# ZhengdiYu/Arbitrary-Hands-3D-Reconstruction

Measured on AMD Instinct MI355X. Metric: frames/sec (2-hand mesh) at 512x512 batch-64; vertex L2 vs ref, higher is better.
Workload: dtype f32; 1 GPU; configs[2]: synthetic 512x512 RGB batch=64 per GPU, HRNet-W32 backbone, fp32; frames_per_gpu=64, global_batch=64, parallelism=frame-sharded x1, gather=none (one rank), contexts_in_turn=2

## Files before the change

### arbitrary-hands-3d-reconstruction_amd/csrc/pair1x1.hip

```cpp
#include "conv_frame.h"

namespace acrmi {

constexpr int PR_C1 = 64, PR_C2 = 256, PR_C3 = 64;
constexpr int PR_PIX = 256;
constexpr int PR_MT = 1, PR_WAVES = PR_PIX / (32 * PR_MT);
constexpr int PR_LDS_FLOATS = PR_C2 * PR_C1 + PR_C3 * PR_C2 + PR_C2 + PR_C3;

__global__ __launch_bounds__(PR_WAVES * 64, 1) void pair1x1_kernel(const float* __restrict__ t2, int t2_cs, int t2_coff,
                                                         const float* __restrict__ x, int x_cs, int x_coff,
                                                         float* __restrict__ y, int y_cs, int y_coff,
                                                         float* __restrict__ t, int t_cs, int t_coff,
                                                         const float* __restrict__ wpk, long npix) {
  extern __shared__ f32x4 smem4[];
  const f32x4* a1 = smem4;
  const f32x4* a2 = smem4 + PR_C2 * PR_C1 / 4;
  const f32x4* b3 = a2 + PR_C3 * PR_C2 / 4;
  const f32x4* b1 = b3 + PR_C2 / 4;
  const int tid = threadIdx.x, lane = tid & 63, wave = tid >> 6;
  const int li = lane & 31, lh = lane >> 5;
  for (int i = tid; i < PR_LDS_FLOATS / 4; i += PR_WAVES * 64) smem4[i] = reinterpret_cast<const f32x4*>(wpk)[i];

  const long items = (npix + PR_PIX - 1) / PR_PIX;
  auto pix_of = [&](long item, int p) -> long { return item * PR_PIX + 32 * PR_MT * wave + 32 * p + li; };
  f32x4 bq[PR_MT][8], bn[PR_MT][8];
  auto request_t2 = [&](long item, f32x4 (&dst)[PR_MT][8]) {
#pragma unroll
    for (int p = 0; p < PR_MT; ++p) {
      long px = pix_of(item, p);
      px = px < npix ? px : npix - 1;
      const f32x4* src = reinterpret_cast<const f32x4*>(t2 + (size_t)px * t2_cs + t2_coff + 32 * lh);
#pragma unroll
      for (int q = 0; q < 8; ++q) dst[p][q] = src[q];
    }
  };
  long item = blockIdx.x;
  if (item < items) request_t2(item, bq);
  __syncthreads();
  for (; item < items; item += gridDim.x) {
    const long nitem = item + gridDim.x;
    if (nitem < items) request_t2(nitem, bn);
    long px[PR_MT];
    bool ok[PR_MT];
#pragma unroll
    for (int p = 0; p < PR_MT; ++p) {
      px[p] = pix_of(item, p);
      ok[p] = px[p] < npix;
      px[p] = ok[p] ? px[p] : npix - 1;
    }
    f32x16 acc2[PR_MT][2];
    const f32x16 zero = {0.f, 0.f, 0.f, 0.f, 0.f, 0.f, 0.f, 0.f, 0.f, 0.f, 0.f, 0.f, 0.f, 0.f, 0.f, 0.f};
#pragma unroll 1
    for (int c = 0; c < 8; ++c) {
      f32x4 rv[PR_MT][4];
#pragma unroll
      for (int p = 0; p < PR_MT; ++p) {
        const float* xr = x + (size_t)px[p] * x_cs + x_coff + 32 * c + 4 * lh;
#pragma unroll
        for (int g = 0; g < 4; ++g) rv[p][g] = *reinterpret_cast<const f32x4*>(xr + 8 * g);
      }
      f32x16 acc1[PR_MT];
#pragma unroll
      for (int s4 = 0; s4 < 8; ++s4) {
        const f32x4 af = a1[(c * 8 + s4) * 64 + lane];
#pragma unroll
        for (int e = 0; e < 4; ++e)
#pragma unroll
          for (int p = 0; p < PR_MT; ++p) {
            if (s4 == 0 && e == 0) acc1[p] = __builtin_amdgcn_mfma_f32_32x32x2f32(af[e], bq[p][s4][e], zero, 0, 0, 0);
            else acc1[p] = __builtin_amdgcn_mfma_f32_32x32x2f32(af[e], bq[p][s4][e], acc1[p], 0, 0, 0);
          }
      }
      f32x4 yv[PR_MT][4];
#pragma unroll
      for (int g = 0; g < 4; ++g) {
        const f32x4 bv = b3[(c * 4 + g) * 2 + lh];
#pragma unroll
        for (int p = 0; p < PR_MT; ++p) {
          f32x4 o = f32x4{acc1[p][4 * g], acc1[p][4 * g + 1], acc1[p][4 * g + 2], acc1[p][4 * g + 3]} + bv + rv[p][g];
          o[0] = fmaxf(o[0], 0.f); o[1] = fmaxf(o[1], 0.f); o[2] = fmaxf(o[2], 0.f); o[3] = fmaxf(o[3], 0.f);
          yv[p][g] = o;
          if (ok[p])
            *reinterpret_cast<f32x4*>(y + (size_t)px[p] * y_cs + y_coff + 32 * c + 8 * g + 4 * lh) = o;
        }
      }
#pragma unroll
      for (int nt = 0; nt < 2; ++nt)
#pragma unroll
        for (int g = 0; g < 4; ++g) {
          const f32x4 af = a2[((c * 2 + nt) * 4 + g) * 64 + lane];
#pragma unroll
          for (int e = 0; e < 4; ++e)
#pragma unroll
            for (int p = 0; p < PR_MT; ++p) {
              if (c == 0 && g == 0 && e == 0) acc2[p][nt] = __builtin_amdgcn_mfma_f32_32x32x2f32(af[e], yv[p][g][e], zero, 0, 0, 0);
              else acc2[p][nt] = __builtin_amdgcn_mfma_f32_32x32x2f32(af[e], yv[p][g][e], acc2[p][nt], 0, 0, 0);
            }
        }
    }
#pragma unroll
    for (int nt = 0; nt < 2; ++nt)
#pragma unroll
      for (int g = 0; g < 4; ++g) {
        const f32x4 bv = b1[(nt * 4 + g) * 2 + lh];
#pragma unroll
        for (int p = 0; p < PR_MT; ++p) {
          f32x4 o = f32x4{acc2[p][nt][4 * g], acc2[p][nt][4 * g + 1], acc2[p][nt][4 * g + 2], acc2[p][nt][4 * g + 3]} + bv;
          o[0] = fmaxf(o[0], 0.f); o[1] = fmaxf(o[1], 0.f); o[2] = fmaxf(o[2], 0.f); o[3] = fmaxf(o[3], 0.f);
          if (ok[p])
            *reinterpret_cast<f32x4*>(t + (size_t)px[p] * t_cs + t_coff + 32 * nt + 8 * g + 4 * lh) = o;
        }
      }
#pragma unroll
    for (int p = 0; p < PR_MT; ++p)
#pragma unroll
      for (int q = 0; q < 8; ++q) bq[p][q] = bn[p][q];
  }
}

hipError_t launch_pair1x1(const float* t2, int t2_cs, int t2_coff, const float* x, int x_cs, int x_coff, float* y, int y_cs,
                          int y_coff, float* t, int t_cs, int t_coff, const float* wpk, long npix, hipStream_t s) {
  if (!t2 || !x || !y || !t || !wpk || npix <= 0 || t2_cs % 4 || x_cs % 4 || y_cs % 4 || t_cs % 4 || t2_coff % 4 || x_coff % 4 ||
      y_coff % 4 || t_coff % 4)
    return hipErrorInvalidValue;
  constexpr size_t lds = (size_t)PR_LDS_FLOATS * sizeof(float);
  static_assert(lds <= 160 * 1024, "both weight matrices must fit the LDS");
  std::lock_guard<std::recursive_mutex> lock(launch_mutex());
  static unsigned char init[MAX_DEVICES] = {};
  if (first_use_on_device(init)) {
    hipError_t e = hipFuncSetAttribute(reinterpret_cast<const void*>(pair1x1_kernel), hipFuncAttributeMaxDynamicSharedMemorySize, (int)lds);
    if (e != hipSuccess) return e;
    if ((e = conv_ensure_device_info()) != hipSuccess) return e;
  }
  const long items = (npix + PR_PIX - 1) / PR_PIX;
  const long cus = conv_num_cus();
  const unsigned grid = (unsigned)(items < cus ? items : cus);
  hipLaunchKernelGGL(pair1x1_kernel, dim3(grid), dim3(PR_WAVES * 64), lds, s, t2, t2_cs, t2_coff, x, x_cs, x_coff, y, y_cs, y_coff, t, t_cs,
                     t_coff, wpk, npix);
  return hipGetLastError();
}

}
```

Before: 2004 frames/s.

## Stage pair1x1 global I/O through per-wave swizzled LDS tiles for coalesced row access

Loads of t2 and the residual x, and stores of y and t, now go through a per-wave 32x32 LDS tile with an XOR swizzle. Each global access becomes a full contiguous row segment instead of a scattered per-pixel gather, and the stores become nontemporal. The next x chunk and the next item's t2 are prefetched into registers, the a1 weight fragment is software-pipelined, and biases are read from global memory so the LDS holds the weights plus one tile per wave. The kernel now requires npix to be a multiple of 256 and channel strides and offsets aligned to 32, and it adds LDS round trips and fills the LDS completely.

```diff
diff --git a/arbitrary-hands-3d-reconstruction_amd/csrc/pair1x1.hip b/arbitrary-hands-3d-reconstruction_amd/csrc/pair1x1.hip
--- a/arbitrary-hands-3d-reconstruction_amd/csrc/pair1x1.hip
+++ b/arbitrary-hands-3d-reconstruction_amd/csrc/pair1x1.hip
@@ -4,8 +4,12 @@
 
 constexpr int PR_C1 = 64, PR_C2 = 256, PR_C3 = 64;
 constexpr int PR_PIX = 256;
-constexpr int PR_MT = 1, PR_WAVES = PR_PIX / (32 * PR_MT);
-constexpr int PR_LDS_FLOATS = PR_C2 * PR_C1 + PR_C3 * PR_C2 + PR_C2 + PR_C3;
+constexpr int PR_WAVES = PR_PIX / 32;
+constexpr int PR_W_FLOATS = PR_C2 * PR_C1 + PR_C3 * PR_C2;
+constexpr int PR_TILE = 32 * 32;
+constexpr int PR_LDS_FLOATS = PR_W_FLOATS + PR_WAVES * PR_TILE;
+
+__device__ __forceinline__ void tile_phase() { asm volatile("" ::: "memory"); }
 
 __global__ __launch_bounds__(PR_WAVES * 64, 1) void pair1x1_kernel(const float* __restrict__ t2, int t2_cs, int t2_coff,
                                                          const float* __restrict__ x, int x_cs, int x_coff,
@@ -15,116 +19,160 @@
   extern __shared__ f32x4 smem4[];
   const f32x4* a1 = smem4;
   const f32x4* a2 = smem4 + PR_C2 * PR_C1 / 4;
-  const f32x4* b3 = a2 + PR_C3 * PR_C2 / 4;
+  const f32x4* b3 = reinterpret_cast<const f32x4*>(wpk + PR_W_FLOATS);
   const f32x4* b1 = b3 + PR_C2 / 4;
-  const int tid = threadIdx.x, lane = tid & 63, wave = tid >> 6;
+  const int tid = threadIdx.x, lane = tid & 63;
+  const int wave = __builtin_amdgcn_readfirstlane(tid >> 6);
   const int li = lane & 31, lh = lane >> 5;
-  for (int i = tid; i < PR_LDS_FLOATS / 4; i += PR_WAVES * 64) smem4[i] = reinterpret_cast<const f32x4*>(wpk)[i];
+  const int p8 = lane >> 3, q8 = lane & 7;
+  float* tile = reinterpret_cast<float*>(smem4) + PR_W_FLOATS + wave * PR_TILE;
+  float* trow = tile + p8 * 32 + 4 * (q8 ^ p8);
+  float* tpix = tile + li * 32;
+  const int sw = li & 7;
+  auto rows_in = [&](const f32x4 (&v)[4]) {
+#pragma unroll
+    for (int gq = 0; gq < 4; ++gq) *reinterpret_cast<f32x4*>(trow + 256 * gq) = v[gq];
+    tile_phase();
+  };
+  auto rows_out = [&](f32x4 (&v)[4]) {
+#pragma unroll
+    for (int gq = 0; gq < 4; ++gq) v[gq] = *reinterpret_cast<const f32x4*>(trow + 256 * gq);
+    tile_phase();
+  };
+  auto pieces_in = [&](const f32x4 (&v)[4]) {
+#pragma unroll
+    for (int g = 0; g < 4; ++g) *reinterpret_cast<f32x4*>(tpix + 4 * ((2 * g + lh) ^ sw)) = v[g];
+    tile_phase();
+  };
+  auto pieces_out = [&](f32x4 (&v)[4]) {
+#pragma unroll
+    for (int g = 0; g < 4; ++g) v[g] = *reinterpret_cast<const f32x4*>(tpix + 4 * ((2 * g + lh) ^ sw));
+    tile_phase();
+  };
+  {
+    constexpr int NST = PR_W_FLOATS / 4 / (PR_WAVES * 64);
+    f32x4 st[NST];
+#pragma unroll
+    for (int i = 0; i < NST; ++i) st[i] = reinterpret_cast<const f32x4*>(wpk)[tid + i * PR_WAVES * 64];
+#pragma unroll
+    for (int i = 0; i < NST; ++i) smem4[tid + i * PR_WAVES * 64] = st[i];
+  }
 
-  const long items = (npix + PR_PIX - 1) / PR_PIX;
-  auto pix_of = [&](long item, int p) -> long { return item * PR_PIX + 32 * PR_MT * wave + 32 * p + li; };
-  f32x4 bq[PR_MT][8], bn[PR_MT][8];
-  auto request_t2 = [&](long item, f32x4 (&dst)[PR_MT][8]) {
+  const long items = npix / PR_PIX;
+  auto row0 = [&](long item, int cs, int coff) -> size_t {
+    return (size_t)(item * PR_PIX + 32 * wave + p8) * (size_t)cs + (size_t)(coff + 4 * q8);
+  };
+  auto request_rows = [&](const float* src, int cs, f32x4 (&dst)[4]) {
 #pragma unroll
-    for (int p = 0; p < PR_MT; ++p) {
-      long px = pix_of(item, p);
-      px = px < npix ? px : npix - 1;
-      const f32x4* src = reinterpret_cast<const f32x4*>(t2 + (size_t)px * t2_cs + t2_coff + 32 * lh);
+    for (int gq = 0; gq < 4; ++gq) dst[gq] = *reinterpret_cast<const f32x4*>(src + (size_t)(8 * gq) * (size_t)cs);
+  };
+  auto store_rows = [&](float* dst, int cs, const f32x4 (&v)[4]) {
 #pragma unroll
-      for (int q = 0; q < 8; ++q) dst[p][q] = src[q];
-    }
+    for (int gq = 0; gq < 4; ++gq) __builtin_nontemporal_store(v[gq], reinterpret_cast<f32x4*>(dst + (size_t)(8 * gq) * (size_t)cs));
   };
+  f32x4 b1v[2][4];
+#pragma unroll
+  for (int nt = 0; nt < 2; ++nt)
+#pragma unroll
+    for (int g = 0; g < 4; ++g) b1v[nt][g] = b1[(nt * 4 + g) * 2 + lh];
+  f32x4 tr[2][4];
+  f32x4 xr[4];
+  f32x4 bq[8];
   long item = blockIdx.x;
-  if (item < items) request_t2(item, bq);
+  if (item < items) {
+    const float* t2r = t2 + row0(item, t2_cs, t2_coff);
+    request_rows(t2r, t2_cs, tr[0]);
+    request_rows(t2r + 32, t2_cs, tr[1]);
+    request_rows(x + row0(item, x_cs, x_coff), x_cs, xr);
+  }
   __syncthreads();
   for (; item < items; item += gridDim.x) {
-    const long nitem = item + gridDim.x;
-    if (nitem < items) request_t2(nitem, bn);
-    long px[PR_MT];
-    bool ok[PR_MT];
+    const long nitem = item + gridDim.x < items ? item + gridDim.x : item;
 #pragma unroll
-    for (int p = 0; p < PR_MT; ++p) {
-      px[p] = pix_of(item, p);
-      ok[p] = px[p] < npix;
-      px[p] = ok[p] ? px[p] : npix - 1;
+    for (int h = 0; h < 2; ++h) {
+      rows_in(tr[h]);
+      if (lh == h) {
+#pragma unroll
+        for (int q = 0; q < 8; ++q) bq[q] = *reinterpret_cast<const f32x4*>(tpix + 4 * (q ^ sw));
+      }
+      tile_phase();
     }
-    f32x16 acc2[PR_MT][2];
+    {
+      const float* t2r = t2 + row0(nitem, t2_cs, t2_coff);
+      request_rows(t2r, t2_cs, tr[0]);
+      request_rows(t2r + 32, t2_cs, tr[1]);
+    }
+    const float* xrow = x + row0(item, x_cs, x_coff);
+    const float* xrow_n = x + row0(nitem, x_cs, x_coff);
+    float* yrow = y + row0(item, y_cs, y_coff);
     const f32x16 zero = {0.f, 0.f, 0.f, 0.f, 0.f, 0.f, 0.f, 0.f, 0.f, 0.f, 0.f, 0.f, 0.f, 0.f, 0.f, 0.f};
+    f32x16 acc2[2] = {zero, zero};
 #pragma unroll 1
     for (int c = 0; c < 8; ++c) {
-      f32x4 rv[PR_MT][4];
+      f32x4 rv[4], bv[4];
 #pragma unroll
-      for (int p = 0; p < PR_MT; ++p) {
-        const float* xr = x + (size_t)px[p] * x_cs + x_coff + 32 * c + 4 * lh;
-#pragma unroll
-        for (int g = 0; g < 4; ++g) rv[p][g] = *reinterpret_cast<const f32x4*>(xr + 8 * g);
-      }
-      f32x16 acc1[PR_MT];
+      for (int g = 0; g < 4; ++g) bv[g] = b3[(c * 4 + g) * 2 + lh];
+      rows_in(xr);
+      pieces_out(rv);
+      request_rows(c < 7 ? xrow + 32 * (c + 1) : xrow_n, x_cs, xr);
+      __builtin_amdgcn_sched_barrier(0);
+      f32x16 acc1;
+      f32x4 afn = a1[(c * 8) * 64 + lane];
 #pragma unroll
       for (int s4 = 0; s4 < 8; ++s4) {
-        const f32x4 af = a1[(c * 8 + s4) * 64 + lane];
+        const f32x4 af = afn;
+        if (s4 < 7) afn = a1[(c * 8 + s4 + 1) * 64 + lane];
 #pragma unroll
-        for (int e = 0; e < 4; ++e)
-#pragma unroll
-          for (int p = 0; p < PR_MT; ++p) {
-            if (s4 == 0 && e == 0) acc1[p] = __builtin_amdgcn_mfma_f32_32x32x2f32(af[e], bq[p][s4][e], zero, 0, 0, 0);
-            else acc1[p] = __builtin_amdgcn_mfma_f32_32x32x2f32(af[e], bq[p][s4][e], acc1[p], 0, 0, 0);
-          }
+        for (int e = 0; e < 4; ++e) {
+          if (s4 == 0 && e == 0) acc1 = __builtin_amdgcn_mfma_f32_32x32x2f32(af[e], bq[s4][e], zero, 0, 0, 0);
+          else acc1 = __builtin_amdgcn_mfma_f32_32x32x2f32(af[e], bq[s4][e], acc1, 0, 0, 0);
+        }
       }
-      f32x4 yv[PR_MT][4];
+      f32x4 yv[4], yr[4];
 #pragma unroll
       for (int g = 0; g < 4; ++g) {
-        const f32x4 bv = b3[(c * 4 + g) * 2 + lh];
+        f32x4 o = f32x4{acc1[4 * g], acc1[4 * g + 1], acc1[4 * g + 2], acc1[4 * g + 3]} + bv[g] + rv[g];
+        o[0] = vrelu1(o[0]); o[1] = vrelu1(o[1]); o[2] = vrelu1(o[2]); o[3] = vrelu1(o[3]);
+        yv[g] = o;
+      }
+      pieces_in(yv);
+      rows_out(yr);
 #pragma unroll
-        for (int p = 0; p < PR_MT; ++p) {
-          f32x4 o = f32x4{acc1[p][4 * g], acc1[p][4 * g + 1], acc1[p][4 * g + 2], acc1[p][4 * g + 3]} + bv + rv[p][g];
-          o[0] = fmaxf(o[0], 0.f); o[1] = fmaxf(o[1], 0.f); o[2] = fmaxf(o[2], 0.f); o[3] = fmaxf(o[3], 0.f);
-          yv[p][g] = o;
-          if (ok[p])
-            *reinterpret_cast<f32x4*>(y + (size_t)px[p] * y_cs + y_coff + 32 * c + 8 * g + 4 * lh) = o;
-        }
-      }
-#pragma unroll
-      for (int nt = 0; nt < 2; ++nt)
+      for (int nt = 0; nt < 2; ++nt) {
 #pragma unroll
         for (int g = 0; g < 4; ++g) {
           const f32x4 af = a2[((c * 2 + nt) * 4 + g) * 64 + lane];
 #pragma unroll
-          for (int e = 0; e < 4; ++e)
+          for (int e = 0; e < 4; ++e) acc2[nt] = __builtin_amdgcn_mfma_f32_32x32x2f32(af[e], yv[g][e], acc2[nt], 0, 0, 0);
+        }
+        if (nt == 0) store_rows(yrow + 32 * c, y_cs, yr);
+      }
+    }
+    float* trow_out = t + row0(item, t_cs, t_coff);
 #pragma unroll
-            for (int p = 0; p < PR_MT; ++p) {
-              if (c == 0 && g == 0 && e == 0) acc2[p][nt] = __builtin_amdgcn_mfma_f32_32x32x2f32(af[e], yv[p][g][e], zero, 0, 0, 0);
-              else acc2[p][nt] = __builtin_amdgcn_mfma_f32_32x32x2f32(af[e], yv[p][g][e], acc2[p][nt], 0, 0, 0);
-            }
-        }
-    }
-#pragma unroll
-    for (int nt = 0; nt < 2; ++nt)
+    for (int nt = 0; nt < 2; ++nt) {
+      f32x4 tv[4], tq[4];
 #pragma unroll
       for (int g = 0; g < 4; ++g) {
-        const f32x4 bv = b1[(nt * 4 + g) * 2 + lh];
-#pragma unroll
-        for (int p = 0; p < PR_MT; ++p) {
-          f32x4 o = f32x4{acc2[p][nt][4 * g], acc2[p][nt][4 * g + 1], acc2[p][nt][4 * g + 2], acc2[p][nt][4 * g + 3]} + bv;
-          o[0] = fmaxf(o[0], 0.f); o[1] = fmaxf(o[1], 0.f); o[2] = fmaxf(o[2], 0.f); o[3] = fmaxf(o[3], 0.f);
-          if (ok[p])
-            *reinterpret_cast<f32x4*>(t + (size_t)px[p] * t_cs + t_coff + 32 * nt + 8 * g + 4 * lh) = o;
-        }
+        f32x4 o = f32x4{acc2[nt][4 * g], acc2[nt][4 * g + 1], acc2[nt][4 * g + 2], acc2[nt][4 * g + 3]} + b1v[nt][g];
+        o[0] = vrelu1(o[0]); o[1] = vrelu1(o[1]); o[2] = vrelu1(o[2]); o[3] = vrelu1(o[3]);
+        tv[g] = o;
       }
-#pragma unroll
-    for (int p = 0; p < PR_MT; ++p)
-#pragma unroll
-      for (int q = 0; q < 8; ++q) bq[p][q] = bn[p][q];
+      pieces_in(tv);
+      rows_out(tq);
+      store_rows(trow_out + 32 * nt, t_cs, tq);
+    }
   }
 }
 
 hipError_t launch_pair1x1(const float* t2, int t2_cs, int t2_coff, const float* x, int x_cs, int x_coff, float* y, int y_cs,
                           int y_coff, float* t, int t_cs, int t_coff, const float* wpk, long npix, hipStream_t s) {
-  if (!t2 || !x || !y || !t || !wpk || npix <= 0 || t2_cs % 4 || x_cs % 4 || y_cs % 4 || t_cs % 4 || t2_coff % 4 || x_coff % 4 ||
-      y_coff % 4 || t_coff % 4)
+  if (!t2 || !x || !y || !t || !wpk || npix <= 0 || npix % PR_PIX || t2_cs % 32 || x_cs % 32 || y_cs % 32 || t_cs % 32 ||
+      t2_coff % 32 || x_coff % 32 || y_coff % 32 || t_coff % 32 || t2_coff < 0 || x_coff < 0 || y_coff < 0 || t_coff < 0 ||
+      t2_coff + PR_C1 > t2_cs || x_coff + PR_C2 > x_cs || y_coff + PR_C2 > y_cs || t_coff + PR_C3 > t_cs)
     return hipErrorInvalidValue;
   constexpr size_t lds = (size_t)PR_LDS_FLOATS * sizeof(float);
-  static_assert(lds <= 160 * 1024, "both weight matrices must fit the LDS");
+  static_assert(lds == 160 * 1024, "both weight matrices and one tile per wave fill the LDS exactly");
   std::lock_guard<std::recursive_mutex> lock(launch_mutex());
   static unsigned char init[MAX_DEVICES] = {};
   if (first_use_on_device(init)) {
@@ -132,7 +180,7 @@
     if (e != hipSuccess) return e;
     if ((e = conv_ensure_device_info()) != hipSuccess) return e;
   }
-  const long items = (npix + PR_PIX - 1) / PR_PIX;
+  const long items = npix / PR_PIX;
   const long cus = conv_num_cus();
   const unsigned grid = (unsigned)(items < cus ? items : cus);
   hipLaunchKernelGGL(pair1x1_kernel, dim3(grid), dim3(PR_WAVES * 64), lds, s, t2, t2_cs, t2_coff, x, x_cs, x_coff, y, y_cs, y_coff, t, t_cs,
```

Measured after the change: 2010 frames/s, median of 6. No clear change (+0.3%).
